# Bioinfo-Tools/PANGEA-plus

Measured on AMD Instinct MI355X. Metric: classified reads/sec (+ HBM GB/s fraction), 150 bp vs 1 Gbp db, 1/2/4/8 GPU, higher is better.
Workload: dtype u64 (2-bit packed bases, integer scores)

## Files before the change

pangea-plus_amd/csrc/classify.hip:

```cpp
#include <algorithm>
#include <chrono>

#include "bitops.hpp"
#include "consensus_core.hpp"
#include "engine.hpp"

namespace pgx {

struct Diag {
	const uint64_t *rw, *ra;
	const uint64_t *dbw, *dba;
	int64_t dstart;
	int lo, hi;
};

template <bool AMB> __device__ __forceinline__ uint64_t mmw(const Diag &D, int w)
{
	int b0 = 32 * w;
	if (b0 + 32 <= D.lo || b0 >= D.hi)
		return kEven;
	uint64_t x = D.rw[w] ^ window64(D.dbw, D.dstart + b0);
	uint64_t m = (x | (x >> 1)) & kEven;
	if (AMB) {
		if (D.ra)
// ... 919 lines not shown
					if (lane == 0)
						base = atomicAdd(&ov.counters[4], (unsigned long long)n);
					base = __shfl(base, 0);
				} else {
					if (chunk_used + n > kChunk) {
						if (lane == 0)
							chunk_base = atomicAdd(&ov.counters[0], (unsigned long long)kChunk);
						chunk_base = __shfl(chunk_base, 0);
						chunk_used = 0;
					}
					base = chunk_base + chunk_used;
					chunk_used += n;
					n_main += lane == 0 ? n : 0;
				}
				pgx_hit *dst = fr ? ov.ovf : ov.main;
				uint8_t *dkey = fr ? ov.ovf_key : ov.main_key;
				const unsigned long long dcap = fr ? ov.ovf_cap : ov.main_cap;
				for (unsigned int i = lane; i < n; i += 64)
					if (base + i < dcap) {
						const pgx_hit hh = RPW == 2 ? (db.gapped ? unpack_seed(st->chit[rs * SLOT_CAP + i], rs ? rB : rA, rs ? wB : wA, rs ? LB : LA)
											  : unpack_hit(st->chit[rs * SLOT_CAP + i], rs ? rB : rA))
									     : st->hit[i];
						dst[base + i] = hh;
						if (db.gapped) {
							dkey[base + i] = seed_key(hh);
							if (!fr)
								ov.main_reg[base + i] = (uint8_t)((uint32_t)hh.sstart >> ov.reg_shift);
						}
					}
				em += n;
				if (!fr)
					start = (uint32_t)base;
			}
			em += st->direct[rs];
			if (lane == 0) {
				read_cnt[rs ? rB : rA] = em;
				read_start[rs ? rB : rA] = start;
			}
		}
		lds_fence();
	}
	for (int d = 32; d >= 1; d >>= 1) {
		n_probe += __shfl_down(n_probe, d);
		n_post += __shfl_down(n_post, d);
		n_runs += __shfl_down(n_runs, d);
	}
	if (lane == 0) {
		atomicAdd(&ov.counters[5], n_main);
		atomicAdd(&ov.counters[6], n_surv);
		atomicAdd(&ov.counters[1], n_probe);
		atomicAdd(&ov.counters[2], n_post);
		atomicAdd(&ov.counters[3], n_runs);
	}
}

constexpr int kScanBlock = 256, kScanItems = 8;

__global__ __launch_bounds__(kScanBlock) void k_scan_partials(const uint32_t *__restrict__ cnt, uint64_t n,
							      uint32_t *__restrict__ partial)
{
	__shared__ uint32_t s[kScanBlock];
	uint64_t base = (uint64_t)blockIdx.x * kScanBlock * kScanItems;
	uint32_t sum = 0;
	for (int k = 0; k < kScanItems; k++) {
		uint64_t i = base + (uint64_t)threadIdx.x * kScanItems + k;
		if (i < n)
			sum += cnt[i];
	}
	s[threadIdx.x] = sum;
	__syncthreads();
	for (int d = kScanBlock / 2; d >= 1; d >>= 1) {
		if ((int)threadIdx.x < d)
			s[threadIdx.x] += s[threadIdx.x + d];
		__syncthreads();
	}
	if (threadIdx.x == 0)
		partial[blockIdx.x] = s[0];
}

__global__ __launch_bounds__(kScanBlock) void k_scan_top(uint32_t *__restrict__ partial, uint32_t n_part)
{
	__shared__ uint32_t s[kScanBlock];
	__shared__ uint32_t carry;
	if (threadIdx.x == 0)
		carry = 0;
	__syncthreads();
	for (uint32_t base = 0; base < n_part; base += kScanBlock) {
		uint32_t i = base + threadIdx.x;
		uint32_t v = i < n_part ? partial[i] : 0;
		s[threadIdx.x] = v;
		__syncthreads();
		for (int d = 1; d < kScanBlock; d <<= 1) {
			uint32_t t = (int)threadIdx.x >= d ? s[threadIdx.x - d] : 0;
			__syncthreads();
			s[threadIdx.x] += t;
			__syncthreads();
		}
		uint32_t incl = s[threadIdx.x];
		if (i < n_part)
			partial[i] = carry + incl - v;
		__syncthreads();
		if (threadIdx.x == kScanBlock - 1)
			carry += incl;
		__syncthreads();
	}
}

__global__ __launch_bounds__(kScanBlock) void k_scan_final(const uint32_t *__restrict__ cnt, uint64_t n,
							   const uint32_t *__restrict__ partial, uint32_t *__restrict__ off)
{
	__shared__ uint32_t s[kScanBlock];
	uint64_t base = (uint64_t)blockIdx.x * kScanBlock * kScanItems;
	uint32_t v[kScanItems], sum = 0;
	for (int k = 0; k < kScanItems; k++) {
		uint64_t i = base + (uint64_t)threadIdx.x * kScanItems + k;
		v[k] = i < n ? cnt[i] : 0;
		sum += v[k];
	}
	s[threadIdx.x] = sum;
	__syncthreads();
	for (int d = 1; d < kScanBlock; d <<= 1) {
		uint32_t t = (int)threadIdx.x >= d ? s[threadIdx.x - d] : 0;
		__syncthreads();
		s[threadIdx.x] += t;
		__syncthreads();
	}
	uint32_t run = partial[blockIdx.x] + s[threadIdx.x] - sum;
	for (int k = 0; k < kScanItems; k++) {
		uint64_t i = base + (uint64_t)threadIdx.x * kScanItems + k;
		if (i < n)
			off[i] = run;
		run += v[k];
	}
	if (blockIdx.x == gridDim.x - 1 && threadIdx.x == kScanBlock - 1)
		off[n] = run;
}

__global__ void k_scatter_hits(const pgx_hit *__restrict__ in, const unsigned long long *__restrict__ n_ptr, unsigned long long in_cap,
			       const uint32_t *__restrict__ off, uint32_t *__restrict__ cursor, pgx_hit *__restrict__ out,
			       unsigned long long out_cap)
{
	const uint64_t n_hits = *n_ptr < in_cap ? *n_ptr : in_cap;
	uint64_t i = (uint64_t)blockIdx.x * blockDim.x + threadIdx.x;
	uint64_t stride = (uint64_t)gridDim.x * blockDim.x;
	for (; i < n_hits; i += stride) {
		pgx_hit h = in[i];
		uint32_t slot = off[h.read] + atomicAdd(&cursor[h.read], 1u);
		if (slot < out_cap)
			out[slot] = h;
	}
}

struct ConsView {
	const uint32_t *subj_tok_off, *subj_tok;
	const int8_t *tok_rank;
	const uint32_t *simrank_lut;
	const uint32_t *simrank_len;
	uint32_t simrank_undef, simrank_zero;
	const uint32_t *rdp_off, *rdp_name;
	const int8_t *rdp_rank;
	const uint8_t *rdp_present;
	const uint32_t *subj_pairs;
	int pair_words;
	const uint32_t *rdp_code;
	int dbg;
	int np_max, nr_max;
};

__device__ __forceinline__ uint32_t hit_simrank(const ConsView &cv, const pgx_hit &h)
{
	const int len = hit_length(h), diffs = hit_diffs(h);
	if (len < 256)
		return cv.simrank_len[len * 256 + diffs];
	return cv.simrank_lut[pident_hundredths(len - diffs, len)];
}

constexpr int kRdpRegs = 8;

template <int NP, int NR>
__device__ __forceinline__ uint32_t pair_grid(const uint32_t (&pr)[15], const uint32_t (&rc)[kRdpRegs], uint32_t np)
{
	uint32_t rm = 0;
#pragma unroll
	for (int a = 0; a < NP; a++) {
		if ((uint32_t)a < np) {
#pragma unroll
			for (int b = 0; b < NR; b++)
				rm += pr[a] == rc[b];
		}
	}
	return rm;
}

__device__ __forceinline__ uint32_t pair_matches(const ConsView &cv, uint32_t subject, const uint32_t (&rc)[kRdpRegs],
						  uint32_t r0, uint32_t r1, uint32_t *ntok_out)
{
#ifdef PGX_STAGE_PROBES
	if (cv.dbg == 7)
		subject &= 0x3FFFu;
#endif
	const uint4 *rec = reinterpret_cast<const uint4 *>(cv.subj_pairs + (unsigned long long)cv.pair_words * subject);
	const uint4 q0 = rec[0];
	const uint4 q1 = rec[1];
	const uint32_t nt = q0.x & 0xFFFFu, np = q0.x >> 16;
	*ntok_out = nt;
	if (np == 0xFFFFu || r1 - r0 > (uint32_t)kRdpRegs) {
		const uint32_t t0 = cv.subj_tok_off[subject], n2 = cv.subj_tok_off[subject + 1] - t0;
		*ntok_out = n2;
		return rank_matches(cv.subj_tok + t0, n2, cv.tok_rank, cv.rdp_name, cv.rdp_rank, r0, r1);
	}
	uint4 q2 = make_uint4(0u, 0u, 0u, 0u), q3 = q2;
	if (cv.pair_words > 8) {
		q2 = rec[2];
		q3 = rec[3];
	}
	const uint32_t pr[15] = { q0.y, q0.z, q0.w, q1.x, q1.y, q1.z, q1.w, q2.x, q2.y, q2.z, q2.w, q3.x, q3.y, q3.z, q3.w };
	if (cv.np_max <= 7 && cv.nr_max <= 6)
		return pair_grid<7, 6>(pr, rc, np);
	return pair_grid<15, kRdpRegs>(pr, rc, np);
}

__device__ __forceinline__ uint32_t hit_rank_matches(const ConsView &cv, uint32_t subject, uint32_t r0, uint32_t r1,
						      uint32_t *ntok_out)
{
	const uint32_t t0 = cv.subj_tok_off[subject], nt = cv.subj_tok_off[subject + 1] - t0;
	*ntok_out = nt;
	return rank_matches(cv.subj_tok + t0, nt, cv.tok_rank, cv.rdp_name, cv.rdp_rank, r0, r1);
}

constexpr uint32_t kNoRead = 0xFFFFFFFFu;
constexpr int kSortCap = 64;

struct SortKey {
	uint64_t k1, k2;
	uint32_t send, mg;
};
__device__ __forceinline__ SortKey make_key(const pgx_hit &h, int best)
{
	SortKey k;
	k.k1 = ((uint64_t)(0xFFFF - best) << 48) | ((uint64_t)(uint32_t)h.subject << 16) | (uint64_t)(0xFFFF - h.score);
	k.k2 = ((uint64_t)(uint32_t)h.qstart << 48) | ((uint64_t)(uint32_t)h.qend << 32) |
	       (uint64_t)(((uint32_t)h.sstart << 1) | (h.send > h.sstart ? 1u : 0u));
	k.send = (uint32_t)h.send;
	k.mg = ((uint32_t)h.mismatch << 16) | (uint32_t)h.gapopen;
	return k;
}

struct SortWave {
	union {
		struct {
			uint64_t k1[kSortCap], k2[kSortCap];
			uint64_t row[kSortCap];
			uint32_t send[kSortCap], mg[kSortCap];
		} a;
		struct {
			uint64_t krm[kSortCap], kcnt[kSortCap];
			uint32_t rm[kSortCap], sim[kSortCap];
		} b;
		struct {
			uint32_t kcnt[kSortCap], sim_e[kSortCap], krm[kSortCap], rm[kSortCap], nxt[kSortCap];
		} c;
	};
	uint32_t rcode[2][kRdpRegs];
};

__device__ __forceinline__ uint64_t order_row(int subject, int score)
{
	return ((uint64_t)(uint32_t)score << 32) | (uint64_t)~(uint32_t)subject;
}

template <int G>
__device__ __forceinline__ uint32_t rank_repeated_subjects(SortWave *sw, const pgx_hit &h, int best, bool mine, int li, int slot0, int lane,
							unsigned long long grp_mask, uint32_t nmax, uint32_t *n_io, bool *dropped_out,
							uint32_t *cnt_out)
{
	uint32_t n = *n_io;
	const SortKey kx = make_key(h, best);
	sw->a.k1[slot0 + li] = mine ? kx.k1 : ~0ull;
	if (mine) {
		sw->a.k2[slot0 + li] = kx.k2;
		sw->a.send[slot0 + li] = kx.send;
		sw->a.mg[slot0 + li] = kx.mg;
	}
	lds_fence();
	bool dropped = false;
	{
		const uint32_t my_s0 = (uint32_t)(h.send > h.sstart ? h.sstart : h.send), my_s1 = (uint32_t)(h.send > h.sstart ? h.send : h.sstart);
		for (uint32_t j = 0; j < nmax; j++) {
			const uint32_t sl = slot0 + (j & (G - 1));
			const uint64_t b1 = sw->a.k1[sl], b2 = sw->a.k2[sl];
			const uint32_t bsend = sw->a.send[sl], bmg = sw->a.mg[sl];
			const bool before = (b1 < kx.k1) | ((b1 == kx.k1) & ((b2 < kx.k2) | ((b2 == kx.k2) & ((bsend < kx.send) | ((bsend == kx.send) &
					    ((bmg < kx.mg) | ((bmg == kx.mg) & (j < (uint32_t)li))))))));
			const bool same = (uint32_t)(b1 >> 16) == (uint32_t)h.subject && ((b2 ^ kx.k2) & 1ull) == 0ull;
			const uint32_t bq0 = (uint32_t)(b2 >> 48), bq1 = (uint32_t)(b2 >> 32) & 0xFFFFu, bsst = (uint32_t)(b2 >> 1) & 0x7FFFFFFFu;
			const uint32_t bs0 = bsend > bsst ? bsst : bsend, bs1 = bsend > bsst ? bsend : bsst;
			const bool dup = (bq0 == (uint32_t)h.qstart && bsst == (uint32_t)h.sstart) || (bq1 == (uint32_t)h.qend && bsend == (uint32_t)h.send) ||
					 ((uint32_t)h.qstart >= bq0 && (uint32_t)h.qend <= bq1 && my_s0 >= bs0 && my_s1 <= bs1);
			dropped |= (j < n) & before & same & dup;
		}
	}
	const unsigned long long drop_mask = __ballot(mine && dropped);
	const uint32_t n_drop = (uint32_t)__popcll(drop_mask & grp_mask);
	const uint32_t n_all = n;
	const bool kept = mine && !dropped;
	if (n_drop) {
		n -= n_drop;
		if (li == 0)
			*cnt_out = n;
	}
	uint32_t rank = 0, same = 0;
	for (uint32_t j0 = 0; j0 < nmax; j0 += 4) {
		uint64_t a1[4];
#pragma unroll
		for (int u = 0; u < 4; u++)
			a1[u] = sw->a.k1[slot0 + ((j0 + u) & (G - 1))];
#pragma unroll
		for (int u = 0; u < 4; u++) {
			const bool in = (j0 + u < n_all) & !((drop_mask >> (slot0 + ((j0 + u) & (G - 1)))) & 1ull);
			rank += (in & (a1[u] < kx.k1)) ? 1u : 0u;
			same += (in & (a1[u] == kx.k1)) ? 1u : 0u;
		}
	}
	if (__ballot(kept && same > 1u)) {
		for (uint32_t j = 0; j < nmax; j++) {
			const uint32_t sl = slot0 + (j & (G - 1));
			const uint64_t b1 = sw->a.k1[sl], b2 = sw->a.k2[sl];
			const uint32_t bsend = sw->a.send[sl], bmg = sw->a.mg[sl];
			const bool before = (b1 == kx.k1) & ((b2 < kx.k2) | ((b2 == kx.k2) & ((bsend < kx.send) | ((bsend == kx.send) &
					    ((bmg < kx.mg) | ((bmg == kx.mg) & (j < (uint32_t)li)))))));
			rank += (before & (j < n_all) & !((drop_mask >> sl) & 1ull)) ? 1u : 0u;
		}
	}
	if (dropped)
		rank = n + (uint32_t)__popcll(drop_mask & grp_mask & ((1ull << lane) - 1ull));
	*n_io = n;
	*dropped_out = dropped;
	return rank;
}

template <int G>
__global__ __launch_bounds__(64 * kWavesPerBlock, 8) void k_sort_consensus(pgx_hit *__restrict__ hits,
									 const pgx_hit *__restrict__ scratch,
									 const uint32_t *__restrict__ read_start,
									 const uint32_t *__restrict__ off, uint32_t *__restrict__ read_cnt,
									 unsigned long long hits_cap, unsigned long long scratch_cap, uint32_t n_reads,
									 const uint32_t *__restrict__ list,
									 const uint32_t *__restrict__ n_list_ptr, ConsView cv,
									 int do_consensus, int lds_ok,
									 pgx_consensus_rec *__restrict__ recs,
									 uint32_t *__restrict__ next_list,
									 uint32_t *__restrict__ next_count)
{
	constexpr int RPW = 64 / G;
	__shared__ SortWave s_sw[kWavesPerBlock];
	const int wave_id = __builtin_amdgcn_readfirstlane((int)(threadIdx.x >> 6));
	SortWave *sw = &s_sw[wave_id];
	const int lane = threadIdx.x & 63;
	const int g = lane / G, li = lane % G, slot0 = g * G;
	const uint32_t total = list ? *n_list_ptr : n_reads;
	uint32_t chunk_base = 0, chunk_used = 64;
	for (uint32_t base = (blockIdx.x * kWavesPerBlock + (uint32_t)wave_id) * RPW; base < total;
	     base += gridDim.x * kWavesPerBlock * RPW) {
		const uint32_t idx = base + (uint32_t)g;
		bool valid = idx < total;
		uint32_t r = valid ? (list ? list[idx] : idx) : 0u;
		if (r == kNoRead) {
			valid = false;
			r = 0;
		}
		const uint32_t o = valid ? off[r] : 0u;
		uint32_t n = valid ? off[r + 1] - o : 0u;
		if ((unsigned long long)o + n > hits_cap)
			n = 0;
		if (valid && n == 0 && do_consensus && li == 0) {
			recs[r].hit = -2;
			recs[r].matches = 0;
		}
		const bool pass_on = valid && (n > (uint32_t)G || !lds_ok);
		if (G == 64) {
			if (pass_on && li == 0)
				next_list[atomicAdd(next_count, 1u)] = r;
		} else {
			const unsigned long long pm = __ballot(pass_on && li == 0);
			if (pm) {
				const uint32_t cnt = (uint32_t)__popcll(pm);
				if (chunk_used + cnt > 64u) {
					if (lane == 0) {
						for (uint32_t k = chunk_used; k < 64u; k++)
							next_list[chunk_base + k] = kNoRead;
						chunk_base = atomicAdd(next_count, 64u);
					}
					chunk_base = __shfl(chunk_base, 0);
					chunk_used = 0;
				}
				if (pass_on && li == 0)
					next_list[chunk_base + chunk_used + (uint32_t)__popcll(pm & ((1ull << lane) - 1))] = r;
				chunk_used += cnt;
			}
		}
		if (pass_on)
			n = 0;
		uint32_t rdp0 = 0, rdp1 = 0, my_code = 0xFFFFFFFEu;
		bool present = true;
		if (do_consensus && n) {
			rdp0 = cv.rdp_off[r];
			rdp1 = cv.rdp_off[r + 1];
			if (li < kRdpRegs && rdp0 + (uint32_t)li < rdp1)
				my_code = cv.rdp_code[rdp0 + (uint32_t)li];
			if (cv.rdp_present)
				present = cv.rdp_present[r] != 0;
		}
		uint32_t st0 = n ? read_start[r] : 0u;
		if (n && st0 != kFragmented && (unsigned long long)st0 + n > scratch_cap) {
			n = 0;
			st0 = 0;
		}
		const pgx_hit *src = st0 == kFragmented ? hits + o : scratch + st0;
		const bool mine = (uint32_t)li < n;
		pgx_hit h;
		h.subject = h.score = h.qstart = h.qend = h.sstart = h.send = h.read = 0;
		h.mismatch = h.gapopen = 0;
		if (mine)
			h = src[li];
		sw->a.row[slot0 + li] = mine ? order_row(h.subject, h.score) : 0ull;
		if (li < kRdpRegs)
			sw->rcode[g][li] = my_code;
		lds_fence();
		if (PGX_SORT_DBG(cv) == 1) {
			if (mine)
				hits[o + li] = h;
			continue;
		}
		const uint32_t nmax = RPW == 2 ? max(__shfl(n, 0), __shfl(n, 32)) : n;
		const uint64_t my_row = order_row(h.subject, h.score);
		int best = h.score;
		uint32_t same_subj = 0;
		uint32_t rank = 0;
		for (uint32_t j0 = 0; j0 < nmax; j0 += 4) {
			uint64_t row[4];
#pragma unroll
			for (int u = 0; u < 4; u++)
				row[u] = sw->a.row[slot0 + ((j0 + u) & (G - 1))];
#pragma unroll
			for (int u = 0; u < 4; u++) {
				rank += row[u] > my_row ? 1u : 0u;
				if ((uint32_t)row[u] == (uint32_t)my_row) {
					same_subj++;
					best = max(best, (int)(row[u] >> 32));
				}
			}
		}
		if (PGX_SORT_DBG(cv) == 2) {
			if (mine) {
				h.score = best;
				hits[o + li] = h;
			}
			continue;
		}
		const unsigned long long grp_mask = G == 64 ? ~0ull : (g ? 0xFFFFFFFF00000000ull : 0x00000000FFFFFFFFull);
		bool dropped = false;
		if (__ballot(mine && same_subj > 1u))
			rank = rank_repeated_subjects<G>(sw, h, best, mine, li, slot0, lane, grp_mask, nmax, &n, &dropped, read_cnt + r);
		const bool kept = mine && !dropped;
		if (mine)
			store_hit_stream(hits + o + rank, h);
		if (!do_consensus || PGX_SORT_DBG(cv) == 3)
			continue;
		uint32_t rmv = 0, ntok = 0, sim = 0;
		if (kept) {
			uint32_t rcode[kRdpRegs];
#pragma unroll
			for (int b = 0; b < kRdpRegs; b++)
				rcode[b] = sw->rcode[g][b];
			sim = hit_simrank(cv, h);
			rmv = pair_matches(cv, (uint32_t)h.subject, rcode, rdp0, rdp1, &ntok);
		}
		if (PGX_SORT_DBG(cv) == 5) {
			if (__ballot(rmv + sim + ntok == 0xFFFFFFF0u) && li == 0)
				recs[r].hit = 0;
			continue;
		}
		const unsigned long long kept_mask = __ballot(kept) & grp_mask;
		const uint32_t c0 = __shfl(ntok, kept_mask ? __ffsll((unsigned long long)kept_mask) - 1 : slot0);
		const bool odd = kept && (ntok != c0 || ntok == 0u || rmv >= 100000000u || sim >= (1u << 25));
		const unsigned long long odd_mask = __ballot(odd);
		const unsigned long long gmask = G == 64 ? ~0ull : (g ? 0xFFFFFFFF00000000ull : 0x00000000FFFFFFFFull);
		const bool slow = (odd_mask & gmask) != 0ull;
		if (n && !present && li == 0) {
			recs[r].hit = -2;
			recs[r].matches = 0;
		}
		const uint32_t k32 = kept ? dec_str_key32(rmv) : 0u;
		uint32_t kmax = k32;
#pragma unroll
		for (int m = 1; m < G; m <<= 1)
			kmax = max(kmax, (uint32_t)__shfl_xor(kmax, m));
		const bool elig = kept && k32 == kmax;
		if (PGX_SORT_DBG(cv) == 6) {
			if (__ballot(elig && slow && !present) && li == 0)
				recs[r].hit = 0;
			continue;
		}
		if (PGX_SORT_DBG(cv) != 4) {
			const uint32_t key2 = elig ? ((sim << 6) | (63u - rank)) + 1u : 0u;
			uint32_t top = key2;
#pragma unroll
			for (int m = 1; m < G; m <<= 1)
				top = max(top, (uint32_t)__shfl_xor(top, m));
			if (elig && key2 == top && present && !slow) {
				recs[r].hit = (int32_t)(o + rank);
				recs[r].matches = (int32_t)rmv;
			}
		}
		if (odd_mask) {
			const bool any_huge = __ballot(kept && (rmv >= 100000000u || ntok >= 100000000u || sim >= (1u << 25))) != 0ull;
			lds_fence();
			if (any_huge) {
				if (kept) {
					sw->b.rm[slot0 + rank] = rmv;
					sw->b.sim[slot0 + rank] = sim;
					sw->b.krm[slot0 + rank] = dec_str_key(rmv);
					sw->b.kcnt[slot0 + rank] = dec_str_key(ntok);
				}
				lds_fence();
				if (li == 0 && n && slow && present) {
					ArgmaxState am;
					am.cursim = r == 0 ? cv.simrank_undef : cv.simrank_zero;
					for (uint32_t k = 0; k < n; k++)
						am.step_keys((int32_t)(o + k), sw->b.rm[slot0 + k], sw->b.krm[slot0 + k], sw->b.kcnt[slot0 + k],
							     sw->b.sim[slot0 + k]);
					recs[r].hit = am.win;
					recs[r].matches = (int32_t)am.maxrm;
				}
			} else {
				const uint32_t c32 = dec_str_key32(ntok);
				if (kept) {
					sw->c.kcnt[slot0 + rank] = c32;
					sw->c.sim_e[slot0 + rank] = sim | (elig ? 0x80000000u : 0u);
					sw->c.krm[slot0 + rank] = k32;
					sw->c.rm[slot0 + rank] = rmv;
				}
				lds_fence();
				if (n && slow && present) {
					const bool top_is_max = (sw->c.sim_e[slot0] >> 31) != 0u;
					const uint32_t init_sim = r == 0 ? cv.simrank_undef : cv.simrank_zero;
					if (top_is_max) {
						uint32_t nx = kNoRead;
						for (uint32_t t = 0; t < n; t++) {
							const uint32_t a = sw->c.kcnt[slot0 + t], b2 = sw->c.sim_e[slot0 + t];
							const bool cand = kept && t > rank && (b2 >> 31) && (a > c32 || (b2 & 0x7FFFFFFFu) > sim);
							nx = (cand && nx == kNoRead) ? t : nx;
						}
						if (kept)
							sw->c.nxt[slot0 + rank] = nx;
						lds_fence();
						if (li == 0) {
							uint32_t w = kNoRead;
							if (sw->c.rm[slot0] > 0u) {
								w = 0;
							} else {
								for (uint32_t t = 0; t < n && w == kNoRead; t++)
									if (sw->c.kcnt[slot0 + t] > 1u  || (sw->c.sim_e[slot0 + t] & 0x7FFFFFFFu) > init_sim)
										w = t;
							}
							if (w != kNoRead) {
								for (uint32_t nxw = sw->c.nxt[slot0 + w]; nxw != kNoRead; nxw = sw->c.nxt[slot0 + w])
									w = nxw;
								recs[r].hit = (int32_t)(o + w);
								recs[r].matches = (int32_t)sw->c.rm[slot0 + w];
							} else {
								recs[r].hit = -1;
								recs[r].matches = 0;
							}
						}
					} else if (li == 0) {
						uint32_t kr = 1u , mrm = 0, kc = 1u, cs = init_sim;
						int32_t win = -1;
						for (uint32_t k = 0; k < n; k++) {
							const uint32_t vkrm = sw->c.krm[slot0 + k], vrm = sw->c.rm[slot0 + k], vkc = sw->c.kcnt[slot0 + k],
								       vs = sw->c.sim_e[slot0 + k] & 0x7FFFFFFFu;
							if (vkrm > kr) {
								kr = vkrm;
								mrm = vrm;
								win = (int32_t)(o + k);
								cs = vs;
							}
							if ((vkc > kc || cs < vs) && vrm == mrm) {
								kc = vkc;
								win = (int32_t)(o + k);
								cs = vs;
							}
						}
						recs[r].hit = win;
						recs[r].matches = (int32_t)mrm;
					}
				}
			}
		}
		lds_fence();
	}
	if (G != 64 && lane == 0 && chunk_used < 64u && chunk_used > 0)
		for (uint32_t k = chunk_used; k < 64u; k++)
			next_list[chunk_base + k] = kNoRead;
}

__global__ void k_consensus_serial(const pgx_hit *__restrict__ hits, const uint32_t *__restrict__ off,
				   const uint32_t *__restrict__ cnt, const uint32_t *__restrict__ list, uint32_t n_list,
				   ConsView cv, pgx_consensus_rec *__restrict__ recs)
{
	uint32_t t = blockIdx.x * blockDim.x + threadIdx.x;
	if (t >= n_list)
		return;
	const uint32_t r = list ? list[t] : t;
	const uint32_t o = off[r], n = cnt[r];
	pgx_consensus_rec rec;
	rec.hit = n ? -1 : -2;
	rec.matches = 0;
	if (cv.rdp_present && !cv.rdp_present[r])
		rec.hit = -2;
	if (rec.hit == -1) {
		const uint32_t r0 = cv.rdp_off[r], r1 = cv.rdp_off[r + 1];
		ArgmaxState am;
		am.cursim = r == 0 ? cv.simrank_undef : cv.simrank_zero;
		for (uint32_t k = 0; k < n; k++) {
			const pgx_hit h = hits[o + k];
			uint32_t c;
			const uint32_t rm = hit_rank_matches(cv, (uint32_t)h.subject, r0, r1, &c);
			am.step((int32_t)(o + k), rm, c, hit_simrank(cv, h));
		}
		rec.hit = am.win;
		rec.matches = (int32_t)am.maxrm;
	}
	recs[r] = rec;
}

__global__ void k_slice_offsets(const uint32_t *__restrict__ off, const uint32_t *__restrict__ cnt, uint32_t first, uint32_t n,
				 uint32_t *__restrict__ off_out, uint32_t *__restrict__ cnt_out)
{
	const uint32_t i = blockIdx.x * blockDim.x + threadIdx.x;
	if (i <= n)
		off_out[i] = off[first + i] - off[first];
	if (i < n)
		cnt_out[i] = cnt[first + i];
}

__global__ void k_slice_hits(const pgx_hit *__restrict__ in, uint64_t base, uint64_t n_slots, uint32_t first, pgx_hit *__restrict__ out)
{
	for (uint64_t i = (uint64_t)blockIdx.x * blockDim.x + threadIdx.x; i < n_slots; i += (uint64_t)gridDim.x * blockDim.x) {
		pgx_hit h = in[base + i];
		h.read -= (int32_t)first;
		out[i] = h;
	}
}

static thread_local pgx_stage_times t_times;

static DbView db_view(const pgx_db *db)
{
	DbView v;
	v.words = db->d_words.data();
	v.amb = db->has_amb ? db->d_amb.data() : nullptr;
	v.seq_off = db->d_seq_off.data();
	v.blk_subj = db->d_blk_subj.data();
	v.blk_info = db->d_blk_info.data();
	v.post_ctx = db->d_post_ctx.data();
	v.amb_blk = db->has_amb ? db->d_amb_blk.data() : nullptr;
	v.bucket_off = db->d_bucket_off.data();
	v.postings = db->d_postings.data();
	v.n_seq = (uint32_t)db->n_seq;
	v.n_bases = db->n_bases;
	v.bits = db->index_bits;
	v.gapped = db->ungapped ? 0 : 1;
	v.deep_from = kGapDeepFrom;
#ifdef PGX_STAGE_PROBES
	v.dbg_stop = getenv("PGX_SEED_STOP") ? atoi(getenv("PGX_SEED_STOP")) : 0;
#else
	v.dbg_stop = 0;
#endif
	return v;
}

static ReadsView reads_view(const pgx_reads *rd)
{
	ReadsView v;
	v.fwd = rd->d_fwd.data();
	v.rc = rd->d_rc.data();
// ... 30 lines not shown
		cv.simrank_zero = db->simrank_zero;
	}
	cv.np_max = db ? db->max_pairs : 15;
	cv.nr_max = rdp ? rdp->max_trip : kRdpRegs;
	if (rdp) {
		cv.rdp_off = rdp->d_off.data();
		cv.rdp_name = rdp->d_name.data();
		cv.rdp_rank = rdp->d_rank.data();
		cv.rdp_present = rdp->d_present.data();
		cv.rdp_code = rdp->d_code.data();
	}
	return cv;
}

struct StageEvents {
	static constexpr int kN = 8;
	hipEvent_t e[kN] = {};
	bool ok = false;
	int init()
	{
		if (ok)
			return 0;
		for (auto &x : e)
			PGX_HIP(hipEventCreate(&x));
		ok = true;
		return 0;
	}
	void mark(int i, hipStream_t s) { (void)hipEventRecord(e[i], s); }
	float ms(int a, int b) const
	{
		float t = 0;
		(void)hipEventElapsedTime(&t, e[a], e[b]);
		return t;
	}
};

__global__ __launch_bounds__(256) void k_merge_pieces(const pgx_hit *__restrict__ scratch, const uint32_t *__restrict__ piece_start,
						      const uint32_t *__restrict__ piece_off, const uint32_t *__restrict__ parent,
						      const uint32_t *__restrict__ qoff, uint32_t n_pieces, pgx_hit *__restrict__ hits,
						      unsigned long long hits_cap, unsigned long long scratch_cap)
{
	const uint32_t waves = gridDim.x * (blockDim.x / 64), lane = threadIdx.x & 63;
	for (uint32_t s = blockIdx.x * (blockDim.x / 64) + (threadIdx.x >> 6); s < n_pieces; s += waves) {
		const uint32_t o = piece_off[s], cnt = piece_off[s + 1] - o;
		if (cnt == 0 || (unsigned long long)o + cnt > hits_cap)
			continue;
		const uint32_t st = piece_start[s];
		if (st != kFragmented && (unsigned long long)st + cnt > scratch_cap)
			continue;
		const pgx_hit *src = st == kFragmented ? hits + o : scratch + st;
		const int32_t read = (int32_t)parent[s], shift = (int32_t)qoff[s];
		for (uint32_t i = lane; i < cnt; i += 64) {
			pgx_hit h = src[i];
			h.read = read;
			h.qstart += shift;
			h.qend += shift;
			hits[o + i] = h;
		}
	}
}

__global__ void k_piece_ranges(const uint32_t *__restrict__ piece_first, const uint32_t *__restrict__ piece_off, uint32_t n_reads,
			       uint32_t *__restrict__ read_off, uint32_t *__restrict__ read_cnt, uint32_t *__restrict__ read_start)
{
	const uint32_t r = blockIdx.x * blockDim.x + threadIdx.x;
	if (r > n_reads)
		return;
	const uint32_t o = piece_off[piece_first[r]];
	read_off[r] = o;
	if (r < n_reads) {
		read_cnt[r] = piece_off[piece_first[r + 1]] - o;
		read_start[r] = kFragmented;
	}
}

struct Workspace {
	hipStream_t stream = nullptr;
	StageEvents ev;
	DevBuf<unsigned long long> counters;
	unsigned long long *h_counters = nullptr;
	DevBuf<pgx_hit> scratch, ovf;
	DevBuf<uint8_t> scratch_key, ovf_key;
	DevBuf<uint8_t> scratch_reg;
	DevBuf<uint32_t> partial, cursor, big_list, read_start, mid_list;
	DevBuf<uint32_t> piece_cnt, piece_off, parent_start;
	DevBuf<pgx_consensus_rec> recs;
	GappedWork gapped;
	DustBufs dust;
	pgx_hits hits;
	uint64_t hit_cap_hint = 0, ovf_cap_hint = 0;
	double table_per_read_hint = 0.0;
	pgx_stage_times times;
	int device = -1;
	~Workspace()
	{
		if (h_counters)
			(void)hipHostFree(h_counters);
		if (stream)
			(void)hipStreamDestroy(stream);
	}
};
constexpr int kNCounters = 12;

static int workspace_of(pgx_db *db, Workspace **out)
{
	if (!db->work) {
		auto w = std::make_shared<Workspace>();
		PGX_HIP(hipGetDevice(&w->device));
		PGX_HIP(hipStreamCreate(&w->stream));
		PGX_HIP(hipHostMalloc((void **)&w->h_counters, (kNCounters + 3) * sizeof(unsigned long long)));
		PGX_TRY(w->ev.init());
		PGX_TRY(w->counters.alloc(kNCounters, 0, 0, true));
		db->work = w;
	}
	*out = static_cast<Workspace *>(db->work.get());
	return 0;
}

int db_stream(pgx_db *db, hipStream_t *out)
{
	Workspace *ws = nullptr;
	PGX_TRY(workspace_of(db, &ws));
	*out = ws->stream;
	return 0;
}

int search_pipeline(pgx_db *db, pgx_reads *rd, const pgx_rdp *rdp, pgx_hits *out, pgx_consensus_rec *d_recs)
{
	PGX_TRY(require_device());
	if (rdp && !db->bound)
		return fail(PGX_E_ARG, "consensus needs pgx_db_bind_taxonomy() first");
	if (rdp && rdp->n != rd->n)
		return fail(PGX_E_ARG, "RDP stream holds %lld reads, batch holds %lld", (long long)rdp->n, (long long)rd->n);
	std::lock_guard<std::mutex> lock(db->search_mu);
	static const bool laps_on = getenv("PGX_CALL_LAPS") != nullptr;
	const auto lap_t0 = std::chrono::steady_clock::now();
	auto lap = [&](const char *what) {
		if (laps_on)
			fprintf(stderr, "[pgx lap] %8.2f ms  %s\n", std::chrono::duration<double, std::milli>(std::chrono::steady_clock::now() - lap_t0).count(), what);
	};
	trace_point("search_pipeline: entered");
	Workspace *wsp = nullptr;
	PGX_TRY(workspace_of(db, &wsp));
	Workspace &ws = *wsp;
	hipStream_t st = ws.stream;
	pgx_stage_times &tm = ws.times;
	memset(&tm, 0, sizeof tm);
	const uint64_t n = (uint64_t)rd->n;
	out->n_reads = rd->n;
	PGX_TRY(out->d_read_cnt.ensure(n + 1));
	PGX_TRY(out->d_read_off.ensure(n + 1));
	if (n == 0) {
		out->n_hits = 0;
		t_times = tm;
		return 0;
	}
	index_check(db, "search_pipeline");
	const DbView dv = db_view(db);
	const bool split = rd->pieces && rd->pieces->n > 0;
	const pgx_reads *sr = split ? rd->pieces.get() : rd;
	const uint64_t ns = (uint64_t)sr->n;
	if (split) {
		PGX_TRY(ws.piece_cnt.ensure(ns + 1));
		PGX_TRY(ws.piece_off.ensure(ns + 1));
		PGX_TRY(ws.parent_start.ensure(n));
	}
	ReadsView rv = reads_view(sr);
	if (!db->dust)
		rv.dustwin_f = rv.dustwin_r = nullptr;
	const int grid = (int)std::min<uint64_t>((n + kWavesPerBlock - 1) / kWavesPerBlock, 256ull * 8);

	uint64_t cap = std::max<uint64_t>(std::max<uint64_t>(std::max(n, ns) * 40, 1 << 16) + 256ull * 8 * kWavesPerBlock * kChunk, ws.hit_cap_hint);
	uint64_t ovf_cap = std::max<uint64_t>(std::max<uint64_t>(std::max(n, ns) / 4, 1 << 16), ws.ovf_cap_hint);
	uint64_t table_cap = std::max<uint64_t>(std::max<uint64_t>(std::max(n, ns) * 36, 1 << 16), (uint64_t)((double)std::max(n, ns) * ws.table_per_read_hint) + 1);
	DevBuf<pgx_hit> &scratch = ws.scratch, &ovf = ws.ovf;
	DevBuf<uint32_t> &read_start = ws.read_start;
	PGX_TRY(read_start.ensure(std::max(n, ns)));
	unsigned long long *h_cnt = ws.h_counters;
	const std::vector<pgx_reads::SearchClass> &classes = sr->classes;
	bool long_reads = false;
	for (auto &c : classes)
		long_reads = long_reads || c.words == 0;
	const uint32_t n_part = (uint32_t)((ns + kScanBlock * kScanItems - 1) / (kScanBlock * kScanItems));
	PGX_TRY(ws.partial.ensure(n_part));
	PGX_TRY(ws.cursor.ensure(ns));
	PGX_TRY(ws.big_list.ensure(n));
	PGX_TRY(ws.mid_list.ensure(n + 64ull * kWavesPerBlock * 256 * 8));
	trace_point("search_pipeline: lists ready");
	const ConsView cv = cons_view(db, rdp);
	const int lds_ok = rd->max_len <= 65535 ? 1 : 0;
	uint64_t H = 0, H_ovf = 0;
	ws.ev.mark(6, st);
	const bool dust_now = db->dust && db->dust_each_search;
	if (dust_now) {
		PGX_TRY(reads_dust_again(sr, ws.dust, st));
		if (sr->has_dust) {
			rv.dustwin_f = ws.dust.win_f.data();
			rv.dustwin_r = ws.dust.win_r.data();
			rv.dust_any = ws.dust.any.data();
		}
	}
	ws.ev.mark(7, st);
	for (int attempt = 0;; attempt++) {
		if (attempt > 8)
			return fail(PGX_E_LIMIT, "hit tables did not settle after %d attempts", attempt);
		PGX_TRY(scratch.ensure(cap));
		PGX_TRY(ovf.ensure(ovf_cap));
		trace_point("search_pipeline: seed tables ready");
		PGX_TRY(out->d_hits.ensure(table_cap));
		trace_point("search_pipeline: hit table ready");
		cap = scratch.n;
		ovf_cap = ovf.n;
		if (dv.gapped) {
			PGX_TRY(ws.scratch_key.ensure(cap + 16));
			PGX_TRY(ws.scratch_reg.ensure(cap + 16));
			PGX_TRY(ws.ovf_key.ensure(ovf_cap));
			PGX_HIP(hipMemsetAsync(ws.scratch_key.data(), 0xFF, cap + 16, st));
		}
		table_cap = out->d_hits.n;
		PGX_HIP(hipMemsetAsync(ws.counters.data(), 0, kNCounters * sizeof(unsigned long long), st));
		OutView ov;
		ov.main = scratch.data();
		ov.ovf = ovf.data();
		ov.main_key = ws.scratch_key.data();
		ov.ovf_key = ws.ovf_key.data();
		ov.main_reg = ws.scratch_reg.data();
		ov.reg_shift = gapped_region_shift(db->n_bases);
		ov.main_cap = cap;
		ov.ovf_cap = ovf_cap;
		ov.counters = ws.counters.data();
		uint32_t *big_count = reinterpret_cast<uint32_t *>(ws.counters.data() + 8), *mid_count = reinterpret_cast<uint32_t *>(ws.counters.data() + 9);
		trace_point("search_pipeline: tables ready");
		lap("tables ready");
		ws.ev.mark(0, st);
		uint32_t *rc_ptr = split ? ws.piece_cnt.data() : out->d_read_cnt.data(), *rs_ptr = read_start.data();
		for (const pgx_reads::SearchClass &c0 : classes) {
			pgx_reads::SearchClass c = c0;
			c.amb = c.amb || db->has_amb;
			ReadsView cvw = rv;
			const uint64_t cn = c.count;
			cvw.n = (uint32_t)cn;
			cvw.list = c.listed ? sr->d_class_list.data() + c.off : nullptr;
			const int per_block = kWavesPerBlock * (c.words > 0 ? 2 : 1);
			const dim3 g((unsigned)std::min<uint64_t>((cn + per_block - 1) / per_block, 256ull * 8)), b(64 * kWavesPerBlock);
#define PGX_SEED_LAUNCH2(A, W, D)                                                                                                  \
	do {                                                                                                                       \
		if (c.listed)                                                                                                      \
			hipLaunchKernelGGL((k_seed_extend<A, W, true, D>), g, b, 0, st, dv, cvw, ov, rc_ptr, rs_ptr);             \
		else                                                                                                               \
			hipLaunchKernelGGL((k_seed_extend<A, W, false, D>), g, b, 0, st, dv, cvw, ov, rc_ptr, rs_ptr);            \
	} while (0)
#define PGX_SEED_LAUNCH(A, W)                                                                                                      \
	do {                                                                                                                       \
		if (c.dust && cvw.dustwin_f)                                                                                       \
			PGX_SEED_LAUNCH2(A, W, true);                                                                              \
		else                                                                                                               \
			PGX_SEED_LAUNCH2(A, W, false);                                                                             \
	} while (0)
			if (c.amb && c.words == 3)
				PGX_SEED_LAUNCH(true, 3);
			else if (c.amb && c.words == 5)
				PGX_SEED_LAUNCH(true, 5);
			else if (c.amb && c.words == 8)
				PGX_SEED_LAUNCH(true, 8);
			else if (c.amb)
				PGX_SEED_LAUNCH(true, 0);
			else if (c.words == 3)
				PGX_SEED_LAUNCH(false, 3);
			else if (c.words == 5)
				PGX_SEED_LAUNCH(false, 5);
			else if (c.words == 8)
				PGX_SEED_LAUNCH(false, 8);
			else
				PGX_SEED_LAUNCH(false, 0);
#undef PGX_SEED_LAUNCH
#undef PGX_SEED_LAUNCH2
		}
		PGX_HIP(hipGetLastError());
		trace_point("k_seed_extend");
		ws.ev.mark(1, st);

		if (dv.gapped) {
			ReadsView all = rv;
			all.n = (uint32_t)ns;
			PGX_TRY(gapped_stage(dv, all, scratch.data(), ws.scratch_key.data(), rs_ptr, rc_ptr, ovf.data(), ws.ovf_key.data(),
					     ws.counters.data() + 4, ovf_cap, long_reads, cap, (int)sr->max_len, ws.gapped, st, ws.counters.data(), ws.scratch_reg.data()));
			trace_point("gapped_stage");
		}
		ws.ev.mark(2, st);

		const uint32_t *unit_cnt = split ? ws.piece_cnt.data() : out->d_read_cnt.data();
		uint32_t *unit_off = split ? ws.piece_off.data() : out->d_read_off.data();
		hipLaunchKernelGGL(k_scan_partials, dim3(n_part), dim3(kScanBlock), 0, st, unit_cnt, ns, ws.partial.data());
		hipLaunchKernelGGL(k_scan_top, dim3(1), dim3(kScanBlock), 0, st, ws.partial.data(), n_part);
		hipLaunchKernelGGL(k_scan_final, dim3(n_part), dim3(kScanBlock), 0, st, unit_cnt, ns, ws.partial.data(), unit_off);
		PGX_HIP(hipMemsetAsync(ws.cursor.data(), 0, ns * sizeof(uint32_t), st));
		hipLaunchKernelGGL(k_scatter_hits, dim3(256), dim3(256), 0, st, ovf.data(), ws.counters.data() + 4, ovf_cap, unit_off,
				   ws.cursor.data(), out->d_hits.data(), table_cap);
		PGX_HIP(hipGetLastError());
		const uint32_t *sort_start = read_start.data();
		if (split) {
			hipLaunchKernelGGL(k_merge_pieces, dim3((unsigned)std::min<uint64_t>((ns + 3) / 4, 256ull * 32)), dim3(256), 0, st, scratch.data(),
					   read_start.data(), ws.piece_off.data(), rd->d_piece_parent.data(), rd->d_piece_qoff.data(), (uint32_t)ns,
					   out->d_hits.data(), table_cap, cap);
			hipLaunchKernelGGL(k_piece_ranges, dim3((unsigned)((n + 1 + 255) / 256)), dim3(256), 0, st, rd->d_piece_first.data(),
					   ws.piece_off.data(), (uint32_t)n, out->d_read_off.data(), out->d_read_cnt.data(), ws.parent_start.data());
			PGX_HIP(hipGetLastError());
			sort_start = ws.parent_start.data();
		}
		trace_point("group");
		ws.ev.mark(3, st);

		const int grid2 = (int)std::min<uint64_t>((n + 2 * kWavesPerBlock - 1) / (2 * kWavesPerBlock), 256ull * 8);
		hipLaunchKernelGGL(k_sort_consensus<32>, dim3(grid2), dim3(64 * kWavesPerBlock), 0, st, out->d_hits.data(), scratch.data(),
				   sort_start, out->d_read_off.data(), out->d_read_cnt.data(), (unsigned long long)table_cap, (unsigned long long)cap, (uint32_t)n,
				   (const uint32_t *)nullptr, (const uint32_t *)nullptr, cv, rdp ? 1 : 0, lds_ok, d_recs, ws.mid_list.data(), mid_count);
		trace_point("k_sort_consensus<32>");
		hipLaunchKernelGGL(k_sort_consensus<64>, dim3(grid), dim3(64 * kWavesPerBlock), 0, st, out->d_hits.data(), scratch.data(),
				   sort_start, out->d_read_off.data(), out->d_read_cnt.data(), (unsigned long long)table_cap, (unsigned long long)cap, (uint32_t)n,
				   ws.mid_list.data(), mid_count, cv, rdp ? 1 : 0, lds_ok, d_recs, ws.big_list.data(), big_count);
		PGX_HIP(hipGetLastError());
		trace_point("k_sort_consensus<64>");
		ws.ev.mark(4, st);

		PGX_HIP(hipMemcpyAsync(h_cnt, ws.counters.data(), kNCounters * sizeof(unsigned long long), hipMemcpyDeviceToHost, st));
		h_cnt[kNCounters] = 0;
		h_cnt[kNCounters + 2] = 0;
		if (dv.gapped) {
			PGX_HIP(hipMemcpyAsync(h_cnt + kNCounters, ws.gapped.big_count.data(), 2 * sizeof(uint32_t), hipMemcpyDeviceToHost, st));
			PGX_HIP(hipMemcpyAsync(h_cnt + kNCounters + 2, ws.gapped.big_count.data() + 4, 2 * sizeof(uint32_t), hipMemcpyDeviceToHost, st));
		}
		PGX_HIP(hipMemcpyAsync(h_cnt + kNCounters + 1, out->d_read_off.data() + n, sizeof(uint32_t), hipMemcpyDeviceToHost, st));
		lap("step enqueued");
		PGX_HIP(hipStreamSynchronize(st));
		lap("step finished");
		H_ovf = h_cnt[4];
		H = h_cnt[5] + H_ovf;
		const uint64_t gap_listed = std::max<uint64_t>((uint32_t)h_cnt[kNCounters], (uint32_t)(h_cnt[kNCounters] >> 32)), gap_cap = ws.gapped.big_list.n;
		bool again = false;
		if (h_cnt[0] > cap) {
			cap = h_cnt[0] + h_cnt[0] / 8;
			again = true;
			tm.grown |= 1;
		}
		if (H_ovf > ovf_cap) {
			ovf_cap = H_ovf + H_ovf / 8;
			again = true;
			tm.grown |= 2;
		}
		if (dv.gapped && gap_listed > gap_cap) {
			PGX_TRY(ws.gapped.big_list.ensure(gap_listed + gap_listed / 8));
			again = true;
			tm.grown |= 4;
		}
		if (!again && H > table_cap) {
			table_cap = H + H / 16;
			again = true;
			tm.grown |= 8;
		}
		tm.attempts = attempt + 1;
		if (!again)
			break;
	}
	ws.hit_cap_hint = std::max<uint64_t>(ws.hit_cap_hint, h_cnt[0] + h_cnt[0] / 16);
	ws.ovf_cap_hint = std::max<uint64_t>(ws.ovf_cap_hint, H_ovf + H_ovf / 16);
	ws.table_per_read_hint = std::max(ws.table_per_read_hint, (double)(H + H / 16) / (double)std::max(n, ns));
	out->n_hits = (int64_t)H;
	out->gapped = dv.gapped != 0;
	tm.hits = (int64_t)H;
	tm.probes = (int64_t)h_cnt[1];
	tm.postings = (int64_t)h_cnt[2];
	tm.candidates = (int64_t)h_cnt[3];
	tm.survivors = (int64_t)h_cnt[6];
	tm.gapped_wide = (int64_t)(uint32_t)h_cnt[kNCounters] + (int64_t)(uint32_t)(h_cnt[kNCounters + 2] >> 32);
	tm.seed_extend_ms = ws.ev.ms(0, 1);
	tm.gapped_ms = ws.ev.ms(1, 2);
	tm.group_ms = ws.ev.ms(2, 3);
	tm.sort_ms = ws.ev.ms(3, 4);
	tm.total_ms = ws.ev.ms(0, 4);
	tm.dust_ms = dust_now ? ws.ev.ms(6, 7) : 0.0f;
	tm.total_ms += tm.dust_ms;
	const unsigned long long hit_limit = getenv("PGX_HIT_LIMIT") ? strtoull(getenv("PGX_HIT_LIMIT"), nullptr, 10) : (1ull << 32);
	if (H >= hit_limit)
		return fail(PGX_E_LIMIT, "%llu hits in one batch exceed the 32-bit slot limit: use smaller batches",
			    (unsigned long long)H);
	const uint32_t n_big = (uint32_t)h_cnt[8];
	if (n_big) {
		const uint32_t *sort_start = split ? ws.parent_start.data() : read_start.data();
		ws.ev.mark(4, st);
		PGX_TRY(sort_big_reads(out->d_hits.data(), scratch.data(), sort_start, out->d_read_off.data(), out->d_read_cnt.data(),
				       ws.big_list.data(), n_big, dv.gapped != 0));
		if (rdp) {
			hipLaunchKernelGGL(k_consensus_serial, dim3((n_big + 63) / 64), dim3(64), 0, 0, out->d_hits.data(), out->d_read_off.data(),
					   out->d_read_cnt.data(), ws.big_list.data(), n_big, cv, d_recs);
			PGX_HIP(hipGetLastError());
		}
		ws.ev.mark(5, 0);
		PGX_HIP(hipDeviceSynchronize());
		const float extra = ws.ev.ms(4, 5);
		tm.sort_ms += extra;
		tm.total_ms += extra;
	}
// ... 186 lines not shown
```

Measured before the change: 126.1 million.

## Precompute compacted read lists by hit count before sort-consensus kernels

Adds a two-pass scan (k_list_partials, k_scan_top run on two segments, k_list_final) that sorts reads into a 32-wide list and a 64-wide list, and writes empty-read consensus records up front. The G=32 sort kernel then runs only over reads that have hits, without the atomic chunked hand-off and the kNoRead padding. It also replaces the rdp range arguments with a sentinel code for reads with many triplets, and hides lane values behind an opaque asm copy to ease register pressure. In exchange, each step launches three extra small kernels and reads the offsets twice.

```diff
diff --git a/pangea-plus_amd/csrc/classify.hip b/pangea-plus_amd/csrc/classify.hip
--- a/pangea-plus_amd/csrc/classify.hip
+++ b/pangea-plus_amd/csrc/classify.hip
@@ -1025,6 +1025,7 @@
 {
 	__shared__ uint32_t s[kScanBlock];
 	__shared__ uint32_t carry;
+	partial += (size_t)blockIdx.x * n_part;
 	if (threadIdx.x == 0)
 		carry = 0;
 	__syncthreads();
@@ -1119,6 +1120,7 @@
 }
 
 constexpr int kRdpRegs = 8;
+constexpr uint32_t kManyTriplets = 0xFFFFFFFDu;
 
 template <int NP, int NR>
 __device__ __forceinline__ uint32_t pair_grid(const uint32_t (&pr)[15], const uint32_t (&rc)[kRdpRegs], uint32_t np)
@@ -1136,7 +1138,7 @@
 }
 
 __device__ __forceinline__ uint32_t pair_matches(const ConsView &cv, uint32_t subject, const uint32_t (&rc)[kRdpRegs],
-						  uint32_t r0, uint32_t r1, uint32_t *ntok_out)
+						  uint32_t read, uint32_t *ntok_out)
 {
 #ifdef PGX_STAGE_PROBES
 	if (cv.dbg == 7)
@@ -1147,10 +1149,10 @@
 	const uint4 q1 = rec[1];
 	const uint32_t nt = q0.x & 0xFFFFu, np = q0.x >> 16;
 	*ntok_out = nt;
-	if (np == 0xFFFFu || r1 - r0 > (uint32_t)kRdpRegs) {
+	if (np == 0xFFFFu || rc[0] == kManyTriplets) {
 		const uint32_t t0 = cv.subj_tok_off[subject], n2 = cv.subj_tok_off[subject + 1] - t0;
 		*ntok_out = n2;
-		return rank_matches(cv.subj_tok + t0, n2, cv.tok_rank, cv.rdp_name, cv.rdp_rank, r0, r1);
+		return rank_matches(cv.subj_tok + t0, n2, cv.tok_rank, cv.rdp_name, cv.rdp_rank, cv.rdp_off[read], cv.rdp_off[read + 1]);
 	}
 	uint4 q2 = make_uint4(0u, 0u, 0u, 0u), q3 = q2;
 	if (cv.pair_words > 8) {
@@ -1212,11 +1214,18 @@
 	return ((uint64_t)(uint32_t)score << 32) | (uint64_t)~(uint32_t)subject;
 }
 
+__device__ __forceinline__ int opaque_copy(int x)
+{
+	asm volatile("" : "+v"(x));
+	return x;
+}
+
 template <int G>
-__device__ __forceinline__ uint32_t rank_repeated_subjects(SortWave *sw, const pgx_hit &h, int best, bool mine, int li, int slot0, int lane,
+__device__ __forceinline__ uint32_t rank_repeated_subjects(SortWave *sw, const pgx_hit &h, int best, bool mine, int lane_in,
 							unsigned long long grp_mask, uint32_t nmax, uint32_t *n_io, bool *dropped_out,
 							uint32_t *cnt_out)
 {
+	const int lane = opaque_copy(lane_in), li = lane % G, slot0 = lane / G * G;
 	uint32_t n = *n_io;
 	const SortKey kx = make_key(h, best);
 	sw->a.k1[slot0 + li] = mine ? kx.k1 : ~0ull;
@@ -1282,12 +1291,91 @@
 	return rank;
 }
 
+__device__ __forceinline__ uint32_t list_class(uint32_t n_hits, int lds_ok)
+{
+	return n_hits == 0 ? 0u : (n_hits <= 32u && lds_ok) ? 1u : 1u << 16;
+}
+
+__global__ __launch_bounds__(kScanBlock) void k_list_partials(const uint32_t *__restrict__ off, uint32_t n, int lds_ok,
+							       uint32_t *__restrict__ partial, uint32_t n_part)
+{
+	__shared__ uint32_t s[kScanBlock];
+	const uint64_t base = (uint64_t)blockIdx.x * kScanBlock * kScanItems + (uint64_t)threadIdx.x * kScanItems;
+	uint32_t sum = 0;
+	if (base < n) {
+		uint32_t lo = off[base];
+		for (int k = 0; k < kScanItems && base + k < n; k++) {
+			const uint32_t hi = off[base + k + 1];
+			sum += list_class(hi - lo, lds_ok);
+			lo = hi;
+		}
+	}
+	s[threadIdx.x] = sum;
+	__syncthreads();
+	for (int d = kScanBlock / 2; d >= 1; d >>= 1) {
+		if ((int)threadIdx.x < d)
+			s[threadIdx.x] += s[threadIdx.x + d];
+		__syncthreads();
+	}
+	if (threadIdx.x == 0) {
+		partial[blockIdx.x] = s[0] & 0xFFFFu;
+		partial[n_part + blockIdx.x] = s[0] >> 16;
+	}
+}
+
+__global__ __launch_bounds__(kScanBlock) void k_list_final(const uint32_t *__restrict__ off, uint32_t n, int lds_ok,
+							    const uint32_t *__restrict__ partial, uint32_t n_part,
+							    uint32_t *__restrict__ list32, uint32_t *__restrict__ list64,
+							    uint32_t *__restrict__ n_list32, uint32_t *__restrict__ n_list64,
+							    pgx_consensus_rec *__restrict__ recs)
+{
+	__shared__ uint32_t s[kScanBlock];
+	const uint64_t base = (uint64_t)blockIdx.x * kScanBlock * kScanItems + (uint64_t)threadIdx.x * kScanItems;
+	uint32_t cls[kScanItems], sum = 0;
+	{
+		uint32_t lo = base < n ? off[base] : 0u;
+		for (int k = 0; k < kScanItems; k++) {
+			cls[k] = 0;
+			if (base + k < n) {
+				const uint32_t hi = off[base + k + 1];
+				cls[k] = list_class(hi - lo, lds_ok);
+				if (hi == lo && recs) {
+					recs[base + k].hit = -2;
+					recs[base + k].matches = 0;
+				}
+				lo = hi;
+			}
+			sum += cls[k];
+		}
+	}
+	s[threadIdx.x] = sum;
+	__syncthreads();
+	for (int d = 1; d < kScanBlock; d <<= 1) {
+		uint32_t t = (int)threadIdx.x >= d ? s[threadIdx.x - d] : 0;
+		__syncthreads();
+		s[threadIdx.x] += t;
+		__syncthreads();
+	}
+	const uint32_t before = s[threadIdx.x] - sum;
+	uint32_t at32 = partial[blockIdx.x] + (before & 0xFFFFu), at64 = partial[n_part + blockIdx.x] + (before >> 16);
+	for (int k = 0; k < kScanItems; k++) {
+		if (cls[k] == 1u)
+			list32[at32++] = (uint32_t)(base + k);
+		else if (cls[k])
+			list64[at64++] = (uint32_t)(base + k);
+	}
+	if (blockIdx.x == gridDim.x - 1 && threadIdx.x == kScanBlock - 1) {
+		*n_list32 = at32;
+		*n_list64 = at64;
+	}
+}
+
 template <int G>
 __global__ __launch_bounds__(64 * kWavesPerBlock, 8) void k_sort_consensus(pgx_hit *__restrict__ hits,
 									 const pgx_hit *__restrict__ scratch,
 									 const uint32_t *__restrict__ read_start,
 									 const uint32_t *__restrict__ off, uint32_t *__restrict__ read_cnt,
-									 unsigned long long hits_cap, unsigned long long scratch_cap, uint32_t n_reads,
+									 unsigned long long hits_cap, unsigned long long scratch_cap,
 									 const uint32_t *__restrict__ list,
 									 const uint32_t *__restrict__ n_list_ptr, ConsView cv,
 									 int do_consensus, int lds_ok,
@@ -1301,56 +1389,31 @@
 	SortWave *sw = &s_sw[wave_id];
 	const int lane = threadIdx.x & 63;
 	const int g = lane / G, li = lane % G, slot0 = g * G;
-	const uint32_t total = list ? *n_list_ptr : n_reads;
-	uint32_t chunk_base = 0, chunk_used = 64;
+	const uint32_t total = *n_list_ptr;
 	for (uint32_t base = (blockIdx.x * kWavesPerBlock + (uint32_t)wave_id) * RPW; base < total;
 	     base += gridDim.x * kWavesPerBlock * RPW) {
 		const uint32_t idx = base + (uint32_t)g;
-		bool valid = idx < total;
-		uint32_t r = valid ? (list ? list[idx] : idx) : 0u;
-		if (r == kNoRead) {
-			valid = false;
-			r = 0;
-		}
+		const bool valid = idx < total;
+		const uint32_t r = valid ? list[idx] : 0u;
 		const uint32_t o = valid ? off[r] : 0u;
 		uint32_t n = valid ? off[r + 1] - o : 0u;
 		if ((unsigned long long)o + n > hits_cap)
 			n = 0;
-		if (valid && n == 0 && do_consensus && li == 0) {
-			recs[r].hit = -2;
-			recs[r].matches = 0;
-		}
-		const bool pass_on = valid && (n > (uint32_t)G || !lds_ok);
 		if (G == 64) {
-			if (pass_on && li == 0)
-				next_list[atomicAdd(next_count, 1u)] = r;
-		} else {
-			const unsigned long long pm = __ballot(pass_on && li == 0);
-			if (pm) {
-				const uint32_t cnt = (uint32_t)__popcll(pm);
-				if (chunk_used + cnt > 64u) {
-					if (lane == 0) {
-						for (uint32_t k = chunk_used; k < 64u; k++)
-							next_list[chunk_base + k] = kNoRead;
-						chunk_base = atomicAdd(next_count, 64u);
-					}
-					chunk_base = __shfl(chunk_base, 0);
-					chunk_used = 0;
-				}
-				if (pass_on && li == 0)
-					next_list[chunk_base + chunk_used + (uint32_t)__popcll(pm & ((1ull << lane) - 1))] = r;
-				chunk_used += cnt;
+			if (n > (uint32_t)G || (n && !lds_ok)) {
+				if (li == 0)
+					next_list[atomicAdd(next_count, 1u)] = r;
+				n = 0;
 			}
 		}
-		if (pass_on)
-			n = 0;
-		uint32_t rdp0 = 0, rdp1 = 0, my_code = 0xFFFFFFFEu;
+		uint32_t my_code = 0xFFFFFFFEu;
 		bool present = true;
 		if (do_consensus && n) {
-			rdp0 = cv.rdp_off[r];
-			rdp1 = cv.rdp_off[r + 1];
+			const uint32_t rdp0 = cv.rdp_off[r], rdp1 = cv.rdp_off[r + 1];
 			if (li < kRdpRegs && rdp0 + (uint32_t)li < rdp1)
 				my_code = cv.rdp_code[rdp0 + (uint32_t)li];
+			if (li == 0 && rdp1 - rdp0 > (uint32_t)kRdpRegs)
+				my_code = kManyTriplets;
 			if (cv.rdp_present)
 				present = cv.rdp_present[r] != 0;
 		}
@@ -1404,7 +1467,7 @@
 		const unsigned long long grp_mask = G == 64 ? ~0ull : (g ? 0xFFFFFFFF00000000ull : 0x00000000FFFFFFFFull);
 		bool dropped = false;
 		if (__ballot(mine && same_subj > 1u))
-			rank = rank_repeated_subjects<G>(sw, h, best, mine, li, slot0, lane, grp_mask, nmax, &n, &dropped, read_cnt + r);
+			rank = rank_repeated_subjects<G>(sw, h, best, mine, lane, grp_mask, nmax, &n, &dropped, read_cnt + r);
 		const bool kept = mine && !dropped;
 		if (mine)
 			store_hit_stream(hits + o + rank, h);
@@ -1417,7 +1480,7 @@
 			for (int b = 0; b < kRdpRegs; b++)
 				rcode[b] = sw->rcode[g][b];
 			sim = hit_simrank(cv, h);
-			rmv = pair_matches(cv, (uint32_t)h.subject, rcode, rdp0, rdp1, &ntok);
+			rmv = pair_matches(cv, (uint32_t)h.subject, rcode, r, &ntok);
 		}
 		if (PGX_SORT_DBG(cv) == 5) {
 			if (__ballot(rmv + sim + ntok == 0xFFFFFFF0u) && li == 0)
@@ -1457,6 +1520,7 @@
 			}
 		}
 		if (odd_mask) {
+			const int lane_o = opaque_copy(lane), li = lane_o % G, slot0 = lane_o / G * G;
 			const bool any_huge = __ballot(kept && (rmv >= 100000000u || ntok >= 100000000u || sim >= (1u << 25))) != 0ull;
 			lds_fence();
 			if (any_huge) {
@@ -1543,9 +1607,6 @@
 		}
 		lds_fence();
 	}
-	if (G != 64 && lane == 0 && chunk_used < 64u && chunk_used > 0)
-		for (uint32_t k = chunk_used; k < 64u; k++)
-			next_list[chunk_base + k] = kNoRead;
 }
 
 __global__ void k_consensus_serial(const pgx_hit *__restrict__ hits, const uint32_t *__restrict__ off,
@@ -1742,7 +1803,8 @@
 	DevBuf<pgx_hit> scratch, ovf;
 	DevBuf<uint8_t> scratch_key, ovf_key;
 	DevBuf<uint8_t> scratch_reg;
-	DevBuf<uint32_t> partial, cursor, big_list, read_start, mid_list;
+	DevBuf<uint32_t> partial, cursor, big_list, read_start;
+	DevBuf<uint32_t> list_partial, pair_list, mid_list;
 	DevBuf<uint32_t> piece_cnt, piece_off, parent_start;
 	DevBuf<pgx_consensus_rec> recs;
 	GappedWork gapped;
@@ -1845,7 +1907,10 @@
 	PGX_TRY(ws.partial.ensure(n_part));
 	PGX_TRY(ws.cursor.ensure(ns));
 	PGX_TRY(ws.big_list.ensure(n));
-	PGX_TRY(ws.mid_list.ensure(n + 64ull * kWavesPerBlock * 256 * 8));
+	const uint32_t n_lpart = (uint32_t)((n + kScanBlock * kScanItems - 1) / (kScanBlock * kScanItems));
+	PGX_TRY(ws.list_partial.ensure(2ull * n_lpart));
+	PGX_TRY(ws.pair_list.ensure(n));
+	PGX_TRY(ws.mid_list.ensure(n));
 	trace_point("search_pipeline: lists ready");
 	const ConsView cv = cons_view(db, rdp);
 	const int lds_ok = rd->max_len <= 65535 ? 1 : 0;
@@ -1889,7 +1954,8 @@
 		ov.main_cap = cap;
 		ov.ovf_cap = ovf_cap;
 		ov.counters = ws.counters.data();
-		uint32_t *big_count = reinterpret_cast<uint32_t *>(ws.counters.data() + 8), *mid_count = reinterpret_cast<uint32_t *>(ws.counters.data() + 9);
+		uint32_t *big_count = reinterpret_cast<uint32_t *>(ws.counters.data() + 8), *mid_count = reinterpret_cast<uint32_t *>(ws.counters.data() + 9),
+			 *pair_count = reinterpret_cast<uint32_t *>(ws.counters.data() + 10);
 		trace_point("search_pipeline: tables ready");
 		lap("tables ready");
 		ws.ev.mark(0, st);
@@ -1971,13 +2037,19 @@
 		trace_point("group");
 		ws.ev.mark(3, st);
 
+		hipLaunchKernelGGL(k_list_partials, dim3(n_lpart), dim3(kScanBlock), 0, st, out->d_read_off.data(), (uint32_t)n, lds_ok,
+				   ws.list_partial.data(), n_lpart);
+		hipLaunchKernelGGL(k_scan_top, dim3(2), dim3(kScanBlock), 0, st, ws.list_partial.data(), n_lpart);
+		hipLaunchKernelGGL(k_list_final, dim3(n_lpart), dim3(kScanBlock), 0, st, out->d_read_off.data(), (uint32_t)n, lds_ok,
+				   ws.list_partial.data(), n_lpart, ws.pair_list.data(), ws.mid_list.data(), pair_count, mid_count, rdp ? d_recs : nullptr);
+		trace_point("read lists");
 		const int grid2 = (int)std::min<uint64_t>((n + 2 * kWavesPerBlock - 1) / (2 * kWavesPerBlock), 256ull * 8);
 		hipLaunchKernelGGL(k_sort_consensus<32>, dim3(grid2), dim3(64 * kWavesPerBlock), 0, st, out->d_hits.data(), scratch.data(),
-				   sort_start, out->d_read_off.data(), out->d_read_cnt.data(), (unsigned long long)table_cap, (unsigned long long)cap, (uint32_t)n,
-				   (const uint32_t *)nullptr, (const uint32_t *)nullptr, cv, rdp ? 1 : 0, lds_ok, d_recs, ws.mid_list.data(), mid_count);
+				   sort_start, out->d_read_off.data(), out->d_read_cnt.data(), (unsigned long long)table_cap, (unsigned long long)cap,
+				   ws.pair_list.data(), pair_count, cv, rdp ? 1 : 0, lds_ok, d_recs, (uint32_t *)nullptr, (uint32_t *)nullptr);
 		trace_point("k_sort_consensus<32>");
 		hipLaunchKernelGGL(k_sort_consensus<64>, dim3(grid), dim3(64 * kWavesPerBlock), 0, st, out->d_hits.data(), scratch.data(),
-				   sort_start, out->d_read_off.data(), out->d_read_cnt.data(), (unsigned long long)table_cap, (unsigned long long)cap, (uint32_t)n,
+				   sort_start, out->d_read_off.data(), out->d_read_cnt.data(), (unsigned long long)table_cap, (unsigned long long)cap,
 				   ws.mid_list.data(), mid_count, cv, rdp ? 1 : 0, lds_ok, d_recs, ws.big_list.data(), big_count);
 		PGX_HIP(hipGetLastError());
 		trace_point("k_sort_consensus<64>");
```

Result: slower. 110.2 million (-12.6%).
